# steventan0110/nFST

Measured on AMD Instinct MI355X. Metric: lattice-arcs/sec forward-backward (log-Z), higher is better.
Workload: dtype f32

## Files before the change

nfst_amd/csrc/fb_kernels.h:

```cpp
#pragma once

struct LdsPlan {
  int rows2, v2, v4;
  __host__ __device__ LdsPlan(int max_rows, int vocab)
      : rows2((max_rows + 1) & ~1), v2((vocab + 3) & ~1), v4((vocab + 3) & ~3) {}
  __host__ __device__ int64_t fb_fixed_precise() const {
    return ((int64_t)2 * rows2 + v2) * 16 + (int64_t)v4 * 4 + 2 * kSweepFlags * 4 + 2048;
  }
  __host__ __device__ int64_t bwd_fixed_precise() const { return ((int64_t)rows2 + v2) * 16 + kSweepFlags * 4 + 1024; }
  static __host__ __device__ int64_t sweep_words(int R, int RS) { return (int64_t)R * kSlotWords + (int64_t)RS * kRawWords; }
  __host__ __device__ int64_t fb_bytes(int R, int RS) const {
    return ((int64_t)2 * rows2 + v2) * 8 + (int64_t)v4 * 4 + 2 * sweep_words(R, RS) * 4 + 2 * kSweepFlags * 4 + 1024;
  }
  __host__ __device__ int64_t bwd_bytes(int R, int RS) const {
    return ((int64_t)rows2 + v2) * 8 + sweep_words(R, RS) * 4 + kSweepFlags * 4;
  }
};


template <int NT, int EXTRA, bool TW = false, bool PREC = false>
__global__ __launch_bounds__(NT) void k_backward(nfst_batch lat, nfst_scores sc, int R, int RS, float *logbeta,
                                                 double *logz64, float *logz32, float2 *beta_me) {
  static_assert(!PREC || TW, "precise flavour: tile waves");
  typedef typename ValOf<PREC>::T VT;
  extern __shared__ float2 lds_raw[];
  VT *lds = reinterpret_cast<VT *>(lds_raw);
  const int b = blockIdx.x, tid = threadIdx.x, lane = tid & 63;
  if (lat.only && lat.only[b] != lat.only_tag) return;
  const float theta_first = tid < lat.vocab ? sc.theta[(size_t)sc.theta_stride * b + tid] : 0.0f;
  const Meta m = load_meta(lat.meta, b);
  const LdsPlan plan(lat.max_rows, lat.vocab);
  VT *beta = lds;
  VT *th = lds + plan.rows2;
  uint32_t *ring = (uint32_t *)(th + plan.v2);
  const Extra ex{lat.weighted ? lat.arc_w : nullptr, sc.arc_scores};
  const int wv = __builtin_amdgcn_readfirstlane(tid >> 6);
  uint32_t *raw = ring + (size_t)R * kSlotWords;
  constexpr int kTwSlot = PREC ? kSlotWordsP : kSlotWords2;
  const int32_t *bwd_perm = lat.bwd_perm + m.bwd_slot_off;
  constexpr bool kSelf = NT != 512;
  constexpr int kAhead = kSelf ? kDmaAheadShared : kDmaAheadDeep;
  constexpr int kNE = kSelf ? 2 : 4, kFirstX = kSelf ? 2 : 4;
  static_assert(!TW || NT == 512, "tile waves: the one-lattice-per-CU flavour");
  if (TW) {
  } else if (kSelf) {
    if (wv == 1) self_start<kAhead>(m.bwd_u, lat.bwd_stream + m.bwd_off, m.bwd_tiles, raw, lane);
  } else if (wv == 2) {
    loader_start(m.bwd_u, lat.bwd_stream + m.bwd_off, m.bwd_tiles, raw, RS, lane);
  }
  const bool x_wave = TW ? (wv == 1 || wv == 2 || wv == 3 || wv == 5) : (EXTRA != 0 && wv >= kFirstX);
  const int x_index = TW ? (wv < 4 ? wv - 1 : 3) : wv - kFirstX;
  WeightWave<8, kNE, EXTRA, TW, PREC> xw8;
  if (x_wave && m.bwd_u == 8) xw8.start_maps(lat.bwd_stream + m.bwd_off, bwd_perm, m.bwd_tiles, ex, x_index, lane);
  for (int i = tid; i < m.n_rows; i += NT) val_set(beta[i], 0.0f, kEZero);
  load_theta(th, sc.theta, sc.theta_stride, b, lat.vocab, tid, NT, theta_first);
  if (x_wave && m.bwd_u == 8) xw8.start_gathers(lane);
  __syncthreads();
  int *flags = (int *)(ring + (TW ? (int64_t)R * kTwSlot : LdsPlan::sweep_words(R, RS)));
  if (tid == 0) {
    val_set(beta[m.sink], 0.5f, 1);
    for (int i = 0; i < kSweepFlags; ++i) flags[i] = 0;
  }
  __syncthreads();
  const bool tw_v2 = TW && m.bwd_wide == 0;
  if (x_wave) {
    run_weights<kNE, EXTRA, TW, PREC>(xw8, m.bwd_u, lat.bwd_stream + m.bwd_off, bwd_perm, m.bwd_tiles, ex, x_index, ring, R, flags,
                                      (const float2 *)th, (const float2 *)beta, tw_v2, lds_addr(flags + kSweepFlags) + lane * (PREC ? 16 : 8), 0u, 0, lane);
  } else if constexpr (TW) {
    if (wv == 0) {
      __builtin_amdgcn_s_setprio(3);
      if constexpr (PREC) tile_sweep2p<kNE>(m.bwd_tiles, ring, R, flags, flags + 4, lane);
      else if (tw_v2) tile_sweep2<4, kNE>(m.bwd_tiles, ring, R, flags, flags + 4, lane);
      else tile_sweep<4, true, kNE>(m.bwd_tiles, ring, R, flags, flags + 4, lane);
      __builtin_amdgcn_s_setprio(0);
    }
  } else if (wv < (kSelf ? 2 : 3))
    run_sweep<EXTRA, kSelf, kAhead, kNE>(wv, m.bwd_u, m.bwd_wide != 0, raw, RS, lat.bwd_stream + m.bwd_off,
              m.bwd_tiles, ring, R, flags, (float2 *)beta, (const float2 *)th, lane);
  __syncthreads();
  if (tid == 0) {
    const double z = me_log64(beta[0]);
    if (logz64) logz64[b] = z;
    if (logz32) logz32[b] = (float)z;
  }
  for (int i = tid; i < m.n_rows; i += NT) {
    if (logbeta) logbeta[m.row_off + i] = me_log32(beta[i]);
    if (beta_me) beta_me[m.row_off + i] = me_f2(beta[i]);
  }
}

__device__ __forceinline__ void exp_me_fast(float extra, float &m, int &e) {
  const float x = fminf(fmaxf(extra, -1.0e8f), 9.0e7f);
  const float kf = rintf(x * 1.44269504088896341f);
  float t = fmaf(-kf, 0.693145751953125f, x);
  t = fmaf(-kf, 1.42860682030941723e-6f, t);
  m = __builtin_amdgcn_exp2f(t * 1.44269504088896341f);
  e = (int)kf;
}
__device__ __forceinline__ float arc_posterior(const float2 av, const float2 bv, const float2 tw, float rz,
                                               int ez, bool has_extra, float mx, int ex) {
  float mw = tw.x;
  int ew = __float_as_int(tw.y);
  if (has_extra) {
    mw *= mx;
    ew += ex;
  }
  const float mm = (av.x * mw) * (bv.x * rz);
  const int ee = __float_as_int(av.y) + ew + __float_as_int(bv.y) - ez;
  return ldexpf(mm, max(ee, -300));
}

template <int NT, int EXTRA, bool FUSED = false, bool TW = false, bool PREC = false>
__global__ __launch_bounds__(NT) void k_forward_backward(
    nfst_batch lat, nfst_scores sc, int R, int RS, float *__restrict__ logalpha, float *__restrict__ logbeta,
    double *__restrict__ logz64, float *__restrict__ logz32, double *__restrict__ logz_total, int total_slot,
    float *__restrict__ posterior,
    float *__restrict__ grad_theta, float2 *__restrict__ beta_me) {
  static_assert(!PREC || (TW && EXTRA != 3), "precise flavour: tile waves, per-arc extras from HBM / L2");
  typedef typename ValOf<PREC>::T VT;
  extern __shared__ float2 lds_raw[];
  VT *lds = reinterpret_cast<VT *>(lds_raw);
  constexpr int kTwSlot = PREC ? kSlotWordsP : kSlotWords2;
  const int b = blockIdx.x, tid = threadIdx.x, lane = tid & 63;
  if (lat.only && lat.only[b] != lat.only_tag) return;
  if (tid == 0) NFST_STAMP(0);
  const float theta_first = tid < lat.vocab ? sc.theta[(size_t)sc.theta_stride * b + tid] : 0.0f;
  const Meta m = load_meta(lat.meta, b);
  const LdsPlan plan(lat.max_rows, lat.vocab);
  VT *alpha = lds;
  VT *beta = lds + plan.rows2;
  VT *th = lds + 2 * plan.rows2;
  float *gth = (float *)(th + plan.v2);
  uint32_t *ring = (uint32_t *)(gth + plan.v4);
  const Extra ex{lat.weighted ? lat.arc_w : nullptr, sc.arc_scores};
  constexpr bool has_extra = EXTRA != 0;
  constexpr bool kCached = EXTRA == 3;
  static_assert(!kCached || TW, "staged extras: tile-wave kernels");
  static_assert(!TW || (NT == 1024 && !FUSED), "tile waves: the one-lattice-per-CU flavour");
  const int wv = __builtin_amdgcn_readfirstlane(tid >> 6);
  const bool bwd_side = (wv & 1) == 0;
  const uint32_t *my_prog = bwd_side ? lat.bwd_stream + m.bwd_off : lat.fwd_stream + m.fwd_off;
  const int32_t *my_perm = bwd_side ? lat.bwd_perm + m.bwd_slot_off : lat.fwd_perm + m.fwd_slot_off;
  const int my_tiles = bwd_side ? m.bwd_tiles : m.fwd_tiles;
  const int my_u = bwd_side ? m.bwd_u : m.fwd_u;
  const bool my_wide = (bwd_side ? m.bwd_wide : m.fwd_wide) != 0;
  uint32_t *my_ring = bwd_side ? ring : ring + (TW ? (int64_t)R * kTwSlot : LdsPlan::sweep_words(R, RS));
  const bool tw_v2 = TW && !my_wide;
  uint32_t *my_raw = my_ring + (size_t)R * kSlotWords;
  constexpr bool kSelf = NT != 1024;
  constexpr int kAhead = kSelf ? kDmaAheadShared : kDmaAheadDeep;
  static_assert(!(FUSED && EXTRA), "the fused sweep takes no per-arc extras");
  static_assert(!(EXTRA && NT < 512), "the extras waves need idle waves: 512 threads at least");
  constexpr int kNE = (TW || NT == 1024) ? 4 : 2, kFirstX = NT == 1024 ? 8 : 4;
  const bool x_wave = TW ? (wv >= 2 && wv < 10) : EXTRA != 0 && wv >= kFirstX;
  const int x_index = TW ? (wv - 2) >> 1 : (wv - kFirstX) >> 1;
  if (FUSED) {
    if (wv < 2) FusedSweep<false>::start(my_prog, my_tiles, lane);
  } else if (TW) {
  } else if (kSelf) {
    if (wv == 2 || wv == 3) self_start<kAhead>(my_u, my_prog, my_tiles, my_raw, lane);
  } else if (wv == 6 || wv == 7) {
    loader_start(my_u, my_prog, my_tiles, my_raw, RS, lane);
  }
  WeightWave<8, kNE, EXTRA, TW, PREC> xw8;
  if (x_wave && my_u == 8) xw8.start_maps(my_prog, my_perm, my_tiles, ex, x_index, lane);
  for (int i = tid; i < m.n_rows; i += NT) {
    val_set(alpha[i], 0.0f, kEZero);
    val_set(beta[i], 0.0f, kEZero);
  }
  load_theta(th, sc.theta, sc.theta_stride, b, lat.vocab, tid, NT, theta_first);
  if (grad_theta) for (int l = tid; l < lat.vocab; l += NT) gth[l] = 0.0f;
  if (x_wave && my_u == 8) xw8.start_gathers(lane);
  __syncthreads();
  int *flags = (int *)(ring + 2 * (TW ? (int64_t)R * kTwSlot : LdsPlan::sweep_words(R, RS)));
  float *xc = (float *)(flags + 2 * kSweepFlags + 256);
  constexpr int kTrash = PREC ? 16 : 8;
  const int xc_first = m.arc_off & ~3;
  if (kCached) {
    const int a_lo = m.arc_off, a_hi = m.arc_off + m.n_arcs;
    for (int a = xc_first + 4 * tid; a < a_hi; a += 4 * NT) {
      float4 x = make_float4(0.0f, 0.0f, 0.0f, 0.0f);
      if (a >= a_lo && a + 4 <= a_hi) {
        if (ex.arc_w) x = *reinterpret_cast<const float4 *>(ex.arc_w + a);
        if (ex.arc_scores) {
          const float4 y = *reinterpret_cast<const float4 *>(ex.arc_scores + a);
          x.x += y.x; x.y += y.y; x.z += y.z; x.w += y.w;
        }
      } else {
        float t[4] = {0.0f, 0.0f, 0.0f, 0.0f};
        for (int q = 0; q < 4; ++q)
          if (a + q >= a_lo && a + q < a_hi) t[q] = ex.at(a + q);
        x = make_float4(t[0], t[1], t[2], t[3]);
      }
      *reinterpret_cast<float4 *>(xc + (a - xc_first)) = x;
    }
  }
  if (tid == 0) {
    val_set(beta[m.sink], 0.5f, 1);
    val_set(alpha[0], 0.5f, 1);
    for (int i = 0; i < 2 * kSweepFlags; ++i) flags[i] = 0;
  }
  __syncthreads();
  if (tid == 0) NFST_STAMP(1);
  const bool want_post = posterior != nullptr || grad_theta != nullptr;
  const int a_begin = m.arc_off, a_end = m.arc_off + m.n_arcs;
  const int v_begin = (a_begin + 3) & ~3, v_end = a_end & ~3;
  constexpr int kSweepThreads = 256;
  constexpr int kHelpers = NT - kSweepThreads;
  constexpr int kPre = (kHelpers > 0) ? 7 : 0;
  uint4 psd[kPre > 0 ? kPre : 1];
  uint2 plb[kPre > 0 ? kPre : 1];
  float4 pxm[kPre > 0 ? kPre : 1];
  int4 pxe[kPre > 0 ? kPre : 1];
  auto extras4 = [&](int a) {
    float4 x = make_float4(0.0f, 0.0f, 0.0f, 0.0f);
    if (kCached) return *reinterpret_cast<const float4 *>(xc + (a - xc_first));
    if (has_extra) {
      if (ex.arc_w) x = *reinterpret_cast<const float4 *>(ex.arc_w + a);
      if (ex.arc_scores) {
        const float4 y = *reinterpret_cast<const float4 *>(ex.arc_scores + a);
        x.x += y.x; x.y += y.y; x.z += y.z; x.w += y.w;
      }
    }
    return x;
  };
  auto preload_arcs = [&]() {
#pragma unroll
    for (int u = 0; u < kPre; ++u) {
      const int a = v_begin + 4 * (u * kHelpers + (tid - kSweepThreads));
      if (a < v_end) {
        psd[u] = *reinterpret_cast<const uint4 *>(lat.arc_sd + a);
        plb[u] = *reinterpret_cast<const uint2 *>(lat.arc_l16 + a);
        if (has_extra) pxm[u] = extras4(a);
      }
    }
    if (has_extra) {
#pragma unroll
      for (int u = 0; u < kPre; ++u) {
        const float4 x = pxm[u];
        exp_me_fast(x.x, pxm[u].x, pxe[u].x); exp_me_fast(x.y, pxm[u].y, pxe[u].y);
        exp_me_fast(x.z, pxm[u].z, pxe[u].z); exp_me_fast(x.w, pxm[u].w, pxe[u].w);
      }
    }
  };
  if constexpr (FUSED) {
    if (wv < 2) {
      const uint32_t trash = lds_addr(flags + 2 * kSweepFlags) + (bwd_side ? 0 : 512) + lane * 8;
      if (my_wide) FusedSweep<true>::run(my_prog, my_tiles, (const float2 *)(bwd_side ? beta : alpha), (const float2 *)th, trash, lane);
      else FusedSweep<false>::run(my_prog, my_tiles, (const float2 *)(bwd_side ? beta : alpha), (const float2 *)th, trash, lane);
    }
  } else if (x_wave) {
    run_weights<kNE, EXTRA, TW, PREC>(xw8, my_u, my_prog, my_perm, my_tiles, ex, x_index, my_ring, R, bwd_side ? flags : flags + kSweepFlags,
                                      (const float2 *)th, (const float2 *)(bwd_side ? beta : alpha), tw_v2,
                                      lds_addr(flags + 2 * kSweepFlags) + (bwd_side ? 0 : 64 * kTrash) + lane * kTrash, lds_addr(xc), xc_first, lane);
    if (TW && wv == 2) NFST_STAMP(6);
  } else if constexpr (TW) {
    if (wv < 2) {
      int *fl = bwd_side ? flags : flags + kSweepFlags;
      __builtin_amdgcn_s_setprio(3);
      if constexpr (PREC) tile_sweep2p<kNE>(my_tiles, my_ring, R, fl, fl + 4, lane);
      else if (tw_v2) tile_sweep2<4, kNE>(my_tiles, my_ring, R, fl, fl + 4, lane, bwd_side ? 5 : -1);
      else tile_sweep<4, true, kNE>(my_tiles, my_ring, R, fl, fl + 4, lane);
      __builtin_amdgcn_s_setprio(0);
      NFST_STAMP(bwd_side ? 2 : 3);
    }
  } else if (wv < 4 || (!kSelf && (wv == 6 || wv == 7))) {
    run_sweep<EXTRA, kSelf, kAhead, kNE>(wv < 4 ? wv >> 1 : 2, my_u, my_wide, my_raw, RS, my_prog,
                     my_tiles, my_ring, R, bwd_side ? flags : flags + kSweepFlags, (float2 *)(bwd_side ? beta : alpha), (const float2 *)th, lane);
  }
  if (kPre > 0 && want_post && tid >= kSweepThreads) preload_arcs();
  __syncthreads();
  if (tid == 0) NFST_STAMP(4);
  const float2 zme = me_f2(beta[0]);
  if (tid == 0) {
    const double z = me_log64(beta[0]);
    if (logz64) logz64[b] = z;
    if (logz_total) {
      atomicAdd(&logz_total[total_slot], z);
      if (b == 0) logz_total[(total_slot + 1) % 3] = 0.0;
    }
    if (logz32) logz32[b] = (float)z;
  }
  const float rz = (zme.x > 0.0f) ? 1.0f / zme.x : 0.0f;
  const int ez = __float_as_int(zme.y);
  auto do_group = [&](const uint4 sd, const uint2 lb, int a, const float4 xm, const int4 xe) {
    const float xmv[4] = {xm.x, xm.y, xm.z, xm.w};
    const int xev[4] = {xe.x, xe.y, xe.z, xe.w};
    const uint32_t sdv[4] = {sd.x, sd.y, sd.z, sd.w};
    const int ll[4] = {(int)(lb.x & 0xffffu), (int)(lb.x >> 16), (int)(lb.y & 0xffffu), (int)(lb.y >> 16)};
    float pp[4];
#pragma unroll
    for (int q = 0; q < 4; ++q) {
      const int s0 = (int)(sdv[q] & 0xffffu), d0 = (int)(sdv[q] >> 16);
      pp[q] = (s0 != d0) ? arc_posterior(me_f2(alpha[s0]), me_f2(beta[d0]), me_f2(th[ll[q]]), rz, ez, has_extra, xmv[q], xev[q]) : 0.0f;
      if (grad_theta && pp[q] > 0.0f) atomicAdd(&gth[ll[q]], pp[q]);
    }
    if (posterior) {
      typedef float f4v __attribute__((ext_vector_type(4)));
      __builtin_nontemporal_store(f4v{pp[0], pp[1], pp[2], pp[3]}, reinterpret_cast<f4v *>(posterior + a));
    }
  };
  if (kPre > 0 && tid >= kSweepThreads && want_post) {
#pragma unroll
    for (int u = 0; u < kPre; ++u) {
      const int a = v_begin + 4 * (u * kHelpers + (tid - kSweepThreads));
      if (a < v_end) do_group(psd[u], plb[u], a, pxm[u], pxe[u]);
    }
  }
  for (int i = tid; i < m.n_rows; i += NT) {
    if (logalpha) __builtin_nontemporal_store(me_log32(alpha[i]), logalpha + m.row_off + i);
    if (logbeta) __builtin_nontemporal_store(me_log32(beta[i]), logbeta + m.row_off + i);
    if (beta_me) beta_me[m.row_off + i] = me_f2(beta[i]);
  }
  if (want_post) {
    constexpr int kPB = 4;
    for (int a0 = v_begin + 4 * (kPre * kHelpers + tid); a0 < v_end; a0 += NT * 4 * kPB) {
      uint4 sd[kPB];
      uint2 lb[kPB];
      float4 xe[kPB];
#pragma unroll
      for (int u = 0; u < kPB; ++u) {
        const int a = min(a0 + u * NT * 4, v_end - 4);
        sd[u] = *reinterpret_cast<const uint4 *>(lat.arc_sd + a);
        lb[u] = *reinterpret_cast<const uint2 *>(lat.arc_l16 + a);
        xe[u] = extras4(a);
      }
#pragma unroll
      for (int u = 0; u < kPB; ++u) {
        const int a = a0 + u * NT * 4;
        if (a >= v_end) break;
        float4 gm = make_float4(1.0f, 1.0f, 1.0f, 1.0f);
        int4 ge = make_int4(0, 0, 0, 0);
        if (has_extra) {
          exp_me_fast(xe[u].x, gm.x, ge.x); exp_me_fast(xe[u].y, gm.y, ge.y);
          exp_me_fast(xe[u].z, gm.z, ge.z); exp_me_fast(xe[u].w, gm.w, ge.w);
        }
        do_group(sd[u], lb[u], a, gm, ge);
      }
    }
    const int n_head = min(v_begin, a_end) - a_begin;
    const int n_tail = (v_end >= v_begin) ? a_end - v_end : 0;
    if (tid < n_head + n_tail) {
      const int a = tid < n_head ? a_begin + tid : v_end + (tid - n_head);
      const int s0 = lat.arc_src[a], d0 = lat.arc_dst[a], l0 = lat.arc_label[a];
      float hm = 1.0f;
      int he = 0;
      if (has_extra) exp_me_fast(kCached ? xc[a - xc_first] : ex.at(a), hm, he);
      const float p = (s0 != d0) ? arc_posterior(me_f2(alpha[s0]), me_f2(beta[d0]), me_f2(th[l0]), rz, ez, has_extra, hm, he) : 0.0f;
      if (posterior) posterior[a] = p;
      if (grad_theta && p > 0.0f) atomicAdd(&gth[l0], p);
    }
    if (grad_theta) {
      __syncthreads();
      float *gout = grad_theta + (size_t)b * lat.vocab;
      for (int l = tid; l < lat.vocab; l += NT) gout[l] = gth[l];
    }
  }
#ifdef NFST_PROF
  __syncthreads();
  if (tid == 0) NFST_STAMP(7);
#endif
}
```

nfst_amd/csrc/tile_pipeline.h:

```cpp
#pragma once

constexpr int kDmaAheadDeep = 8, kRawSlotsDeep = 12, kDmaAheadShared = 4, kRawSlotsShared = kDmaAheadShared + 1;
constexpr int kRawWords = 64 * (1 + 4);
constexpr int kSlotWords = 64 * (1 + 3 * 4);
constexpr int kSlotWords2 = 1024;
constexpr int kSlotWordsP = 1280;
constexpr int kPreciseTiles = 192;
constexpr int kMaxRing = 12, kMinRing = 3;

template <int CTRL>
__device__ __forceinline__ int dpp_i(int v) {
  return __builtin_amdgcn_update_dpp(0, v, CTRL, 0xf, 0xf, false);
}
template <int CTRL>
__device__ __forceinline__ float dpp_f(float v) {
  return __int_as_float(__builtin_amdgcn_update_dpp(0, __float_as_int(v), CTRL, 0xf, 0xf, false));
}

template <int STAGES>
__device__ __forceinline__ int seg_max(int Em, int g) {
  if (STAGES >= 1) { const int o = dpp_i<0xB1>(Em); Em = (g >= 1) ? max(Em, o) : Em; }
  if (STAGES >= 2) { const int o = dpp_i<0x4E>(Em); Em = (g >= 2) ? max(Em, o) : Em; }
  if (STAGES >= 3) { const int o = dpp_i<0x141>(Em); Em = (g >= 3) ? max(Em, o) : Em; }
  if (STAGES >= 4) { const int o = dpp_i<0x140>(Em); Em = (g >= 4) ? max(Em, o) : Em; }
// ... 837 lines not shown
}

constexpr int kSweepFlags = 8;
template <int EXTRA, bool SELF, int AHEAD, int NE>
__device__ __forceinline__ void run_sweep(int role, int U, bool wide, uint32_t *raw, int RS, const uint32_t *g,
                                          int n_tiles, uint32_t *ring, int R, int *flags,
                                          float2 *val, const float2 *th, int lane) {
  int *prog = flags, *land = flags + 1, *rland = flags + 2, *xland = flags + 4;
  if (role == 0) {
    if (U == 8) U = 4;
    if (wide) {
      if (U == 4) tile_sweep<4, true>(n_tiles, ring, R, prog, land, lane);
      else if (U == 2) tile_sweep<2, true>(n_tiles, ring, R, prog, land, lane);
      else tile_sweep<1, true>(n_tiles, ring, R, prog, land, lane);
    } else {
      if (U == 4) tile_sweep<4, false>(n_tiles, ring, R, prog, land, lane);
      else if (U == 2) tile_sweep<2, false>(n_tiles, ring, R, prog, land, lane);
      else tile_sweep<1, false>(n_tiles, ring, R, prog, land, lane);
    }
  } else if (role == 1) {
    if (U == 8) tile_decoder<8, EXTRA, SELF, AHEAD>(n_tiles, raw, RS, rland, g, xland, NE, ring, R, prog, land, val, th, lane);
    else if (U == 4) tile_decoder<4, EXTRA, SELF, AHEAD>(n_tiles, raw, RS, rland, g, xland, NE, ring, R, prog, land, val, th, lane);
    else if (U == 2) tile_decoder<2, EXTRA, SELF, AHEAD>(n_tiles, raw, RS, rland, g, xland, NE, ring, R, prog, land, val, th, lane);
    else tile_decoder<1, EXTRA, SELF, AHEAD>(n_tiles, raw, RS, rland, g, xland, NE, ring, R, prog, land, val, th, lane);
  } else if (role == 2) {
    if (!SELF) {
      if (U == 8) tile_loader<8, AHEAD>(g, n_tiles, raw, RS, land, rland, lane);
      else if (U == 4) tile_loader<4, AHEAD>(g, n_tiles, raw, RS, land, rland, lane);
      else if (U == 2) tile_loader<2, AHEAD>(g, n_tiles, raw, RS, land, rland, lane);
      else tile_loader<1, AHEAD>(g, n_tiles, raw, RS, land, rland, lane);
    }
  }
}

template <int U>
struct Dec2 {
  uint32_t dst;
  float k0, k1, k2;
  uint32_t opa[U];
  v2f tw[U];
};
template <int U>
__device__ __forceinline__ void dec2_fetch(uint32_t sb, int lane, Dec2<U> &d) {
  const v4u h = *(const lds_v4u *)(uintptr_t)(sb + lane * 16);
  d.dst = h.x; d.k0 = __uint_as_float(h.y); d.k1 = __uint_as_float(h.z); d.k2 = __uint_as_float(h.w);
  if (U == 4) {
    const v4u a = *(const lds_v4u *)(uintptr_t)(sb + 1024 + lane * 16);
    const v4f p = *(const lds_v4f *)(uintptr_t)(sb + 2048 + lane * 16);
    const v4f q = *(const lds_v4f *)(uintptr_t)(sb + 3072 + lane * 16);
    d.opa[0] = a.x; d.opa[1 % U] = a.y; d.opa[2 % U] = a.z; d.opa[3 % U] = a.w;
    d.tw[0] = v2f{p.x, p.y}; d.tw[1 % U] = v2f{p.z, p.w}; d.tw[2 % U] = v2f{q.x, q.y}; d.tw[3 % U] = v2f{q.z, q.w};
  } else if (U == 2) {
    const v2u a = *(const lds_v2u *)(uintptr_t)(sb + 1024 + lane * 8);
    const v4f p = *(const lds_v4f *)(uintptr_t)(sb + 2048 + lane * 16);
    d.opa[0] = a.x; d.opa[1 % U] = a.y;
    d.tw[0] = v2f{p.x, p.y}; d.tw[1 % U] = v2f{p.z, p.w};
  } else {
    d.opa[0] = *(const lds_u32 *)(uintptr_t)(sb + 1024 + lane * 4);
    d.tw[0] = *(const lds_v2f *)(uintptr_t)(sb + 2048 + lane * 8);
  }
}
template <int U>
__device__ __forceinline__ void tile_math2(const v2f (&tw)[U], const v2f (&vv)[U], const Dec2<U> &c, int &ref) {
  const int nref = -ref;
  float mt[U];
  int d[U];
#pragma unroll
  for (int j = 0; j < U; ++j) {
    mt[j] = tw[j].x * vv[j].x;
    d[j] = __float_as_int(tw[j].y) + __float_as_int(vv[j].y) + nref;
  }
  int dmax = d[0];
#pragma unroll
  for (int j = 1; j < U; ++j) dmax = max(dmax, d[j]);
  float M = ldexpf(mt[0], d[0]);
#pragma unroll
  for (int j = 1; j < U; ++j) M += ldexpf(mt[j], d[j]);
  constexpr int kZeroish = -(1 << 27);
  const bool bad = ((uint32_t)(dmax + 64) > 128u) & (dmax > kZeroish);
  int E = ref;
  const int e0 = __builtin_amdgcn_readfirstlane(dmax);
  const int ref_old = ref;
  ref = (e0 > kZeroish) ? e0 + ref_old : ref_old;
  if (__builtin_expect(__builtin_amdgcn_ballot_w64(bad) != 0, 0)) {
    M = ldexpf(mt[0], d[0] - dmax);
#pragma unroll
    for (int j = 1; j < U; ++j) M += ldexpf(mt[j], d[j] - dmax);
    E = dmax + ref_old;
    const uint64_t m0 = __builtin_amdgcn_ballot_w64(c.k0 != 0.0f), m1 = __builtin_amdgcn_ballot_w64(c.k1 != 0.0f),
                   m2 = __builtin_amdgcn_ballot_w64(c.k2 != 0.0f);
    seg_reduce_exec<3>(M, E, m0, m1, m2);
  } else {
    asm volatile(
        "s_nop 1\n\t"
        "v_fmac_f32_dpp %[m], %[m], %[k0] quad_perm:[1,0,3,2] row_mask:0xf bank_mask:0xf\n\t"
        "s_nop 1\n\t"
        "v_fmac_f32_dpp %[m], %[m], %[k1] quad_perm:[2,3,0,1] row_mask:0xf bank_mask:0xf\n\t"
        "s_nop 1\n\t"
        "v_fmac_f32_dpp %[m], %[m], %[k2] row_half_mirror row_mask:0xf bank_mask:0xf"
        : [m] "+v"(M)
        : [k0] "v"(c.k0), [k1] "v"(c.k1), [k2] "v"(c.k2));
    E = (M == 0.0f) ? kEZero : E;
  }
  const float2 r = me_pack(M, E);
  *(lds_v2f *)(uintptr_t)c.dst = v2f{r.x, r.y};
}

template <int U>
__device__ __forceinline__ int tile_math3(const Dec2<U> &c, const v2f (&vv)[U], const int ref) {
  const int nref = -ref;
  float mt[U];
  int d[U];
#pragma unroll
  for (int j = 0; j < U; ++j) {
    mt[j] = c.tw[j].x * vv[j].x;
    asm("v_add3_u32 %0, %1, %2, %3" : "=v"(d[j]) : "v"(__float_as_int(c.tw[j].y)), "v"(__float_as_int(vv[j].y)), "s"(nref));
  }
  int dmax = d[0];
#pragma unroll
  for (int j = 1; j < U; ++j) dmax = max(dmax, d[j]);
  constexpr int kZeroish = -(1 << 27);
  const uint64_t bad = __builtin_amdgcn_ballot_w64(((uint32_t)(dmax + 64) > 128u) & (dmax > kZeroish));
  const int ref_old = ref;
  float M = ldexpf(mt[0], d[0]);
#pragma unroll
  for (int j = 1; j < U; ++j) M += ldexpf(mt[j], d[j]);
  asm volatile(
      "s_nop 1\n\t"
      "v_fmac_f32_dpp %[m], %[m], %[k0] quad_perm:[1,0,3,2] row_mask:0xf bank_mask:0xf\n\t"
      "s_nop 1\n\t"
      "v_fmac_f32_dpp %[m], %[m], %[k1] quad_perm:[2,3,0,1] row_mask:0xf bank_mask:0xf\n\t"
      "s_nop 1\n\t"
      "v_fmac_f32_dpp %[m], %[m], %[k2] row_half_mirror row_mask:0xf bank_mask:0xf"
      : [m] "+v"(M)
      : [k0] "v"(c.k0), [k1] "v"(c.k1), [k2] "v"(c.k2));
  int E = ref_old;
  if (__builtin_expect(bad != 0, 0)) {
    M = ldexpf(mt[0], d[0] - dmax);
#pragma unroll
    for (int j = 1; j < U; ++j) M += ldexpf(mt[j], d[j] - dmax);
    E = dmax + ref_old;
    const uint64_t m0 = __builtin_amdgcn_ballot_w64(c.k0 != 0.0f), m1 = __builtin_amdgcn_ballot_w64(c.k1 != 0.0f),
                   m2 = __builtin_amdgcn_ballot_w64(c.k2 != 0.0f);
    seg_reduce_exec<3>(M, E, m0, m1, m2);
  }
  int ex;
  const float mant = frexpf(M, &ex);
  const int eo = (M != 0.0f) ? max(E + ex, kEZero) : kEZero;
  *(lds_v2f *)(uintptr_t)c.dst = v2f{mant, __int_as_float(eo)};
  return dmax;
}

#ifdef NFST_PROF
__device__ unsigned long long fb_prof[4096 * 8];
#define NFST_STAMP(k) do { if ((threadIdx.x & 63) == 0 && blockIdx.x < 4096) fb_prof[blockIdx.x * 8 + (k)] = wall_clock64(); } while (0)
#else
#define NFST_STAMP(k) do { } while (0)
#endif
template <int U, int NEF>
__device__ __forceinline__ void tile_sweep2(int n_tiles, const uint32_t *ring, int R, int *prog, const int *land, int lane, int prof_slot = -1) {
  static_assert(NEF == 4, "four tile waves per sweep");
  (void)prof_slot;
  if (n_tiles <= 0) return;
  constexpr uint32_t SB = kSlotWords2 * 4;
  const uint32_t ring_base = lds_addr(ring), ring_end = ring_base + (uint32_t)R * SB;
  const uint32_t land_a = lds_addr(land), prog_a = lds_addr(prog);
  auto flags_now = [&]() { return *(const volatile lds_v4u *)(uintptr_t)land_a; };
  auto margin_x = [](const v4u f) { return min(min((int)f.y - 1, (int)f.z - 2), (int)f.w - 3); };
  auto margin_y = [](const v4u f) { return (int)f.x - 4; };
  auto wait_group = [&](int T, int which) {
    for (;;) {
      const v4u f = flags_now();
      if (__builtin_amdgcn_readfirstlane(which ? margin_y(f) : margin_x(f)) > T) break;
      __builtin_amdgcn_s_sleep(1);
    }
    asm volatile("" ::: "memory");
  };
  while (__builtin_amdgcn_readfirstlane((int)*(const volatile lds_u32 *)(uintptr_t)land_a) <= 0) __builtin_amdgcn_s_sleep(1);
  asm volatile("" ::: "memory");
#ifdef NFST_PROF
  if (prof_slot >= 0) NFST_STAMP(prof_slot);
#endif
  uint32_t gbase = ring_base;
  v4u margin = {0u, 0u, 0u, 0u}, margin1 = {0u, 0u, 0u, 0u};
  int ref = 0;
  int dmax0 = 0;
  Dec2<U> da, db;
  dec2_fetch<U>(gbase, lane, da);
  asm volatile("" ::: "memory");
#define NFST_S2_STEP(K, CUR, NXT)                                                                          \
  {                                                                                                       \
    v2f vv[U];                                                                                            \
    _Pragma("unroll") for (int j = 0; j < U; ++j) vv[j] = *(const lds_v2f *)(uintptr_t)CUR.opa[j];         \
    asm volatile("" ::: "memory");                                                                        \
    __builtin_amdgcn_sched_barrier(0);          \
    if (K == 3) {                                                                                         \
      gbase = (gbase + 4 * SB == ring_end) ? ring_base : gbase + 4 * SB;                                  \
      asm volatile("" ::"v"(margin1));                                                                    \
      if (__builtin_expect(__builtin_amdgcn_readfirstlane(margin_y(margin1)) <= T, 0)) wait_group(T, 1);     \
    }                                                                                                     \
    dec2_fetch<U>(gbase + (K == 3 ? 0u : (K + 1) * SB), lane, NXT);                                       \
    if (K == 1) margin1 = flags_now();                                                                     \
    if (K == 3) margin = flags_now();                                                        \
    asm volatile("" ::: "memory");                                                                        \
    __builtin_amdgcn_sched_barrier(0);                                                                    \
    const int dm_ = tile_math3<U>(CUR, vv, ref);                                                          \
    if (K == 0) dmax0 = dm_;                                                                              \
    if (K & 1) *(volatile lds_u32 *)(uintptr_t)prog_a = (uint32_t)(T + K + 2);  \
    asm volatile("" ::: "memory");                                                                        \
    __builtin_amdgcn_sched_barrier(0);                                                                    \
  }
  int T = 0;
  for (; T + 4 <= n_tiles; T += 4) {
    asm volatile("" ::"v"(margin));
    if (__builtin_expect(__builtin_amdgcn_readfirstlane(margin_x(margin)) <= T, 0)) wait_group(T, 0);
    NFST_S2_STEP(0, da, db)
    NFST_S2_STEP(1, db, da)
    NFST_S2_STEP(2, da, db)
    NFST_S2_STEP(3, db, da)
    const int e0 = __builtin_amdgcn_readfirstlane(dmax0);
    ref = __builtin_amdgcn_readfirstlane((e0 > -(1 << 27)) ? e0 + ref : ref);
  }
  if (T < n_tiles) {
    asm volatile("" ::"v"(margin));
    if (__builtin_expect(__builtin_amdgcn_readfirstlane(margin_x(margin)) <= T, 0)) wait_group(T, 0);
    NFST_S2_STEP(0, da, db)
    if (T + 1 < n_tiles) {
      NFST_S2_STEP(1, db, da)
      if (T + 2 < n_tiles) NFST_S2_STEP(2, da, db)
    }
  }
#undef NFST_S2_STEP
}

struct Dec2P {
  uint32_t dst;
  uint32_t k0, k1, k2;
  uint32_t opa[4];
  double wm[4];
  int we[4];
};
__device__ __forceinline__ void dec2p_fetch(uint32_t sb, int lane, Dec2P &d) {
  const v4u h = *(const lds_v4u *)(uintptr_t)(sb + lane * 16);
  const v4u a = *(const lds_v4u *)(uintptr_t)(sb + 1024 + lane * 16);
  const v4u p = *(const lds_v4u *)(uintptr_t)(sb + 2048 + lane * 16);
  const v4u q = *(const lds_v4u *)(uintptr_t)(sb + 3072 + lane * 16);
  const v4u e = *(const lds_v4u *)(uintptr_t)(sb + 4096 + lane * 16);
  d.dst = h.x; d.k0 = h.y; d.k1 = h.z; d.k2 = h.w;
  d.opa[0] = a.x; d.opa[1] = a.y; d.opa[2] = a.z; d.opa[3] = a.w;
  d.wm[0] = __hiloint2double((int)p.y, (int)p.x); d.wm[1] = __hiloint2double((int)p.w, (int)p.z);
  d.wm[2] = __hiloint2double((int)q.y, (int)q.x); d.wm[3] = __hiloint2double((int)q.w, (int)q.z);
  d.we[0] = (int)e.x; d.we[1] = (int)e.y; d.we[2] = (int)e.z; d.we[3] = (int)e.w;
}
template <int CTRL>
__device__ __forceinline__ double dpp_d(double v) {
  return __hiloint2double(__builtin_amdgcn_update_dpp(0, __double2hiint(v), CTRL, 0xf, 0xf, false),
                          __builtin_amdgcn_update_dpp(0, __double2loint(v), CTRL, 0xf, 0xf, false));
}
template <int STAGES>
__device__ __forceinline__ double seg_sum64(double M, int g) {
  if (STAGES >= 1) { const double o = dpp_d<0xB1>(M); M = (g >= 1) ? M + o : M; }
  if (STAGES >= 2) { const double o = dpp_d<0x4E>(M); M = (g >= 2) ? M + o : M; }
  if (STAGES >= 3) { const double o = dpp_d<0x141>(M); M = (g >= 3) ? M + o : M; }
  if (STAGES >= 4) { const double o = dpp_d<0x140>(M); M = (g >= 4) ? M + o : M; }
  if (STAGES >= 5) { const double o = __shfl_xor(M, 16); M = (g >= 5) ? M + o : M; }
  if (STAGES >= 6) { const double o = __shfl_xor(M, 32); M = (g >= 6) ? M + o : M; }
  return M;
}
__device__ __forceinline__ double ldexp_clamped(double m, int d) {
  return ldexp(m, max(d, -2000));
}
__device__ __forceinline__ int tile_math3p(const Dec2P &c, const Rec64 (&vv)[4], const int ref) {
  const int nref = -ref;
  double mt[4];
  int d[4];
#pragma unroll
  for (int j = 0; j < 4; ++j) {
    mt[j] = c.wm[j] * vv[j].m;
    asm("v_add3_u32 %0, %1, %2, %3" : "=v"(d[j]) : "v"(c.we[j]), "v"(vv[j].e), "s"(nref));
  }
  int dmax = d[0];
#pragma unroll
  for (int j = 1; j < 4; ++j) dmax = max(dmax, d[j]);
  constexpr int kZeroish = -(1 << 27);
  const uint32_t wide = (c.dst >> 25) & 1u;
  const uint64_t bad = __builtin_amdgcn_ballot_w64((((uint32_t)(dmax + 900) > 1800u) & (dmax > kZeroish)) | (wide != 0));
  double M = ldexp(mt[0], d[0]);
#pragma unroll
  for (int j = 1; j < 4; ++j) M += ldexp(mt[j], d[j]);
  {
    int plo, phi;
#define NFST_DPP_PAIR(CTRL)                                                                                              \
    asm volatile("s_nop 1\n\tv_mov_b32_dpp %0, %2 " CTRL " row_mask:0xf bank_mask:0xf\n\tv_mov_b32_dpp %1, %3 " CTRL      \
                 " row_mask:0xf bank_mask:0xf" : "=&v"(plo), "=&v"(phi) : "v"(__double2loint(M)), "v"(__double2hiint(M)))
    NFST_DPP_PAIR("quad_perm:[1,0,3,2]");
    M = fma(__hiloint2double(phi, plo), __hiloint2double((int)c.k0, 0), M);
    NFST_DPP_PAIR("quad_perm:[2,3,0,1]");
    M = fma(__hiloint2double(phi, plo), __hiloint2double((int)c.k1, 0), M);
    NFST_DPP_PAIR("row_half_mirror");
    M = fma(__hiloint2double(phi, plo), __hiloint2double((int)c.k2, 0), M);
#undef NFST_DPP_PAIR
  }
  int E = ref;
  if (__builtin_expect(bad != 0, 0)) {
    const int g = (int)ctl_g(c.dst);
    M = ldexp_clamped(mt[0], d[0] - dmax);
#pragma unroll
    for (int j = 1; j < 4; ++j) M += ldexp_clamped(mt[j], d[j] - dmax);
// ... 145 lines not shown
```

profiles/tune/chunk_stamps.py:

```python
import ctypes as C, os, sys
sys.path.insert(0, os.path.dirname(os.path.dirname(os.path.dirname(os.path.abspath(__file__)))))
import numpy as np, torch
from nfst_amd import ops, synth, _lib
from nfst_amd.lattice import LatticeBatch
B = int(sys.argv[1]) if len(sys.argv) > 1 else 64
dev = torch.device("cuda")
if len(sys.argv) > 2 and sys.argv[2] == "narrow":
    sys.path.insert(0, os.path.dirname(os.path.abspath(__file__)))
    rng = np.random.default_rng(8000)
    lats = [synth.layered_lattice(8000 + i, n_states=int(rng.integers(400, 1501)), avg_degree=float(rng.choice([3.0, 5.0])), vocab=250,
                                  width=int(rng.choice([1, 2, 3])), span=int(rng.choice([1, 2])), max_degree=40) for i in range(B)]
else:
    lats = synth.snips_shaped_batch(B, vocab=250)
host = LatticeBatch.from_synth(lats)
assert host.build_chunks(force=True)
lat = host.to(dev)
theta = torch.from_numpy(synth.label_scores(1, 250, mean=-1.5, std=0.8)).to(dev)
for _ in range(5):
    r = ops.forward_backward(lat, theta)
torch.cuda.synchronize()
raw = C.CDLL(_lib.LIB_PATH)
n = 2 * B
buf = np.zeros(n * 8, np.uint64)
assert raw.nfst_prof_read(buf.ctypes.data_as(C.c_void_p), n * 8) == 0
t = buf.reshape(n, 8).astype(np.int64)
own = (t[:, 1:5] - t[:, :4]) / 100.0
rel_end = (t[:, 4] - t[:, 0].min()) / 100.0
m = lat.chunks.meta_host.reshape(n, 8)
tab = lat.chunks._t["tab"].cpu().numpy().reshape(-1, 4)
longest = np.array([tab[m[i, 4]:m[i, 4] + m[i, 0], 2].max() for i in range(n)])
print("us per phase (median / max over workgroups): weights+init %.1f / %.1f, pass 1 %.1f / %.1f, pass 2 %.1f / %.1f, pass 3 %.1f / %.1f; last end %.1f" %
      (np.median(own[:, 0]), own[:, 0].max(), np.median(own[:, 1]), own[:, 1].max(), np.median(own[:, 2]), own[:, 2].max(),
       np.median(own[:, 3]), own[:, 3].max(), rel_end.max()))
print("pass 1: ns per entry of the longest chunk: median %.0f min %.0f max %.0f" % tuple(np.percentile(own[:, 1] * 1e3 / longest, [50, 0, 100])))
print("pass 2: ns per chunk: median %.0f; by F:" % np.median(own[:, 2] * 1e3 / m[:, 0]),
      {int(F): round(float(np.median((own[:, 2] * 1e3 / m[:, 0])[m[:, 1] == F]))) for F in np.unique(m[:, 1])})
slow = np.argsort(rel_end)[-4:]
print("slowest:", [(int(i), "C %d F %d R %d longest %d" % (m[i, 0], m[i, 1], m[i, 2], longest[i]), [round(float(x), 1) for x in own[i]]) for i in slow])
```

profiles/tune/stamps.py:

```python
import ctypes as C, os, sys
sys.path.insert(0, os.path.dirname(os.path.dirname(os.path.dirname(os.path.abspath(__file__)))))
import numpy as np, torch
from nfst_amd import ops, synth, _lib
from nfst_amd.lattice import LatticeBatch
B = int(sys.argv[1]) if len(sys.argv) > 1 else 256
rot = int(sys.argv[2]) if len(sys.argv) > 2 else 4
dev = torch.device("cuda")
lats = [LatticeBatch.from_synth(synth.bench_batch(B, first_seed=1234 + 100000 * r), device=dev) for r in range(rot)]
theta = torch.from_numpy(synth.label_scores(1, 256)).to(dev)
outs = [None] * rot
for it in range(10 * rot + 1):
    r = it % rot
    outs[r] = ops.forward_backward(lats[r], theta, out=outs[r])
torch.cuda.synchronize()
raw = C.CDLL(_lib.LIB_PATH)
buf = np.zeros(B * 8, np.uint64)
assert raw.nfst_prof_read(buf.ctypes.data_as(C.c_void_p), B * 8) == 0
t = buf.reshape(B, 8).astype(np.int64)
rel = (t - t[:, 0].min()) / 100.0
lat = lats[0]
tiles = np.maximum(lat.meta_host[:, _lib.META_BWD_TILES], lat.meta_host[:, _lib.META_FWD_TILES])
names = ["entry", "init done", "beta swept", "alpha swept", "barrier", "first tile", "tile wave 0 done", "end"]
print(f"B={B}, {rot} batches rotating: us since the first workgroup entered (min / median / max over workgroups)")
for i in (0, 1, 5, 6, 2, 3, 4, 7):
    print(f"  {names[i]:18s} {rel[:, i].min():8.2f} {np.median(rel[:, i]):8.2f} {rel[:, i].max():8.2f}")
own = (t - t[:, :1]) / 100.0
print("  per workgroup, since its own entry: init %.2f, first tile %.2f, sweeps done %.2f, barrier -> end %.2f (medians)" %
      (np.median(own[:, 1]), np.median(own[:, 5]), np.median(np.maximum(own[:, 2], own[:, 3])), np.median(own[:, 7] - own[:, 4])))
dur = (np.maximum(t[:, 2], t[:, 3]) - t[:, 5]) / 100.0
print("  sweep duration / tile (ns): min %.0f median %.0f max %.0f;  tiles: min %d median %d max %d" %
      (*np.percentile(dur / tiles * 1e3, [0, 50, 100]), tiles.min(), np.median(tiles), tiles.max()))
slow = np.argsort(rel[:, 7])[-4:]
print("  slowest workgroups (id, tiles, first tile, swept, end):", [(int(b), int(tiles[b]), round(float(rel[b, 5]), 2), round(float(max(rel[b, 2], rel[b, 3])), 2), round(float(rel[b, 7]), 2)) for b in slow])
```

Measured before the change: 131.0 billion.

## Use buffer stores for outputs, vectorize row logs, rebalance sweep/helper threads

Posterior and log-alpha/log-beta outputs now go through raw buffer-resource 128-bit stores with a streaming cache policy. The row log outputs are written four at a time with an aligned head and tail, and the alpha and beta rows start at different thread offsets. The fused kernel also reserves 128 instead of 256 threads for the sweep, giving more threads to posterior preloading with 6 prefetched groups each. Extra profiling stamps are added. Risks: fewer sweep-side threads may slow the sweep phase, and buffer bounds or alignment handling could be wrong at row edges.

```diff
diff --git a/nfst_amd/csrc/fb_kernels.h b/nfst_amd/csrc/fb_kernels.h
--- a/nfst_amd/csrc/fb_kernels.h
+++ b/nfst_amd/csrc/fb_kernels.h
@@ -86,6 +86,36 @@
   for (int i = tid; i < m.n_rows; i += NT) {
     if (logbeta) logbeta[m.row_off + i] = me_log32(beta[i]);
     if (beta_me) beta_me[m.row_off + i] = me_f2(beta[i]);
+  }
+}
+
+typedef float f4v __attribute__((ext_vector_type(4)));
+struct OutBuf {
+  __amdgpu_buffer_rsrc_t rsrc;
+  __device__ __forceinline__ OutBuf(float *p, int n_floats) {
+    const uint64_t a = (uint64_t)(uintptr_t)p;
+    const uint32_t lo = __builtin_amdgcn_readfirstlane((uint32_t)a), hi = __builtin_amdgcn_readfirstlane((uint32_t)(a >> 32));
+    rsrc = __builtin_amdgcn_make_buffer_rsrc(reinterpret_cast<void *>((uintptr_t)(((uint64_t)hi << 32) | lo)), 0,
+                                             __builtin_amdgcn_readfirstlane(n_floats) * 4, 0x00020000);
+  }
+  __device__ __forceinline__ void store4(int i, const f4v v) const {
+    typedef uint32_t u4v __attribute__((ext_vector_type(4)));
+    __builtin_amdgcn_raw_buffer_store_b128(__builtin_bit_cast(u4v, v), rsrc, i * 4, 0, 16);
+  }
+};
+template <int NT, class VT>
+__device__ __forceinline__ void rows_out(float *out, const VT *val, int n, int tid, int first) {
+  const int head = min((int)((0u - (uint32_t)(uintptr_t)out) >> 2 & 3u), n);
+  const int groups = (n - head) >> 2, tail = head + 4 * groups;
+  const OutBuf ob(out, n);
+  for (int g = (tid - first) & (NT - 1); g < groups; g += NT) {
+    const int i = head + 4 * g;
+    ob.store4(i, f4v{me_log32(val[i]), me_log32(val[i + 1]), me_log32(val[i + 2]), me_log32(val[i + 3])});
+  }
+  const int t = (tid - first) & (NT - 1);
+  if (t < head + (n - tail)) {
+    const int i = t < head ? t : tail + (t - head);
+    __builtin_nontemporal_store(me_log32(val[i]), out + i);
   }
 }
 
@@ -205,9 +235,9 @@
   const bool want_post = posterior != nullptr || grad_theta != nullptr;
   const int a_begin = m.arc_off, a_end = m.arc_off + m.n_arcs;
   const int v_begin = (a_begin + 3) & ~3, v_end = a_end & ~3;
-  constexpr int kSweepThreads = 256;
+  constexpr int kSweepThreads = 128;
   constexpr int kHelpers = NT - kSweepThreads;
-  constexpr int kPre = (kHelpers > 0) ? 7 : 0;
+  constexpr int kPre = (NT > 256) ? 6 : 0;
   uint4 psd[kPre > 0 ? kPre : 1];
   uint2 plb[kPre > 0 ? kPre : 1];
   float4 pxm[kPre > 0 ? kPre : 1];
@@ -283,6 +313,7 @@
   }
   const float rz = (zme.x > 0.0f) ? 1.0f / zme.x : 0.0f;
   const int ez = __float_as_int(zme.y);
+  const OutBuf post_out(posterior ? posterior + a_begin : nullptr, posterior ? m.n_arcs : 0);
   auto do_group = [&](const uint4 sd, const uint2 lb, int a, const float4 xm, const int4 xe) {
     const float xmv[4] = {xm.x, xm.y, xm.z, xm.w};
     const int xev[4] = {xe.x, xe.y, xe.z, xe.w};
@@ -295,10 +326,7 @@
       pp[q] = (s0 != d0) ? arc_posterior(me_f2(alpha[s0]), me_f2(beta[d0]), me_f2(th[ll[q]]), rz, ez, has_extra, xmv[q], xev[q]) : 0.0f;
       if (grad_theta && pp[q] > 0.0f) atomicAdd(&gth[ll[q]], pp[q]);
     }
-    if (posterior) {
-      typedef float f4v __attribute__((ext_vector_type(4)));
-      __builtin_nontemporal_store(f4v{pp[0], pp[1], pp[2], pp[3]}, reinterpret_cast<f4v *>(posterior + a));
-    }
+    if (posterior) post_out.store4(a - a_begin, f4v{pp[0], pp[1], pp[2], pp[3]});
   };
   if (kPre > 0 && tid >= kSweepThreads && want_post) {
 #pragma unroll
@@ -307,11 +335,17 @@
       if (a < v_end) do_group(psd[u], plb[u], a, pxm[u], pxe[u]);
     }
   }
-  for (int i = tid; i < m.n_rows; i += NT) {
-    if (logalpha) __builtin_nontemporal_store(me_log32(alpha[i]), logalpha + m.row_off + i);
-    if (logbeta) __builtin_nontemporal_store(me_log32(beta[i]), logbeta + m.row_off + i);
-    if (beta_me) beta_me[m.row_off + i] = me_f2(beta[i]);
-  }
+#ifdef NFST_PROF
+  if (wv == 4) {
+    NFST_STAMP(8);
+    asm volatile("s_waitcnt vmcnt(0)" ::: "memory");
+    NFST_STAMP(9);
+  }
+#endif
+  if (logalpha) rows_out<NT>(logalpha + m.row_off, alpha, m.n_rows, tid, 0);
+  if (logbeta) rows_out<NT>(logbeta + m.row_off, beta, m.n_rows, tid, NT / 2);
+  if (beta_me) for (int i = tid; i < m.n_rows; i += NT) beta_me[m.row_off + i] = me_f2(beta[i]);
+  if (wv == 0) NFST_STAMP(10);
   if (want_post) {
     constexpr int kPB = 4;
     for (int a0 = v_begin + 4 * (kPre * kHelpers + tid); a0 < v_end; a0 += NT * 4 * kPB) {
diff --git a/nfst_amd/csrc/tile_pipeline.h b/nfst_amd/csrc/tile_pipeline.h
--- a/nfst_amd/csrc/tile_pipeline.h
+++ b/nfst_amd/csrc/tile_pipeline.h
@@ -1013,8 +1013,9 @@
 }
 
 #ifdef NFST_PROF
-__device__ unsigned long long fb_prof[4096 * 8];
-#define NFST_STAMP(k) do { if ((threadIdx.x & 63) == 0 && blockIdx.x < 4096) fb_prof[blockIdx.x * 8 + (k)] = wall_clock64(); } while (0)
+constexpr int kProfSlots = 16;
+__device__ unsigned long long fb_prof[4096 * kProfSlots];
+#define NFST_STAMP(k) do { if ((threadIdx.x & 63) == 0 && blockIdx.x < 4096) fb_prof[blockIdx.x * kProfSlots + (k)] = wall_clock64(); } while (0)
 #else
 #define NFST_STAMP(k) do { } while (0)
 #endif
diff --git a/profiles/tune/chunk_stamps.py b/profiles/tune/chunk_stamps.py
--- a/profiles/tune/chunk_stamps.py
+++ b/profiles/tune/chunk_stamps.py
@@ -21,9 +21,9 @@
 torch.cuda.synchronize()
 raw = C.CDLL(_lib.LIB_PATH)
 n = 2 * B
-buf = np.zeros(n * 8, np.uint64)
-assert raw.nfst_prof_read(buf.ctypes.data_as(C.c_void_p), n * 8) == 0
-t = buf.reshape(n, 8).astype(np.int64)
+buf = np.zeros(n * 16, np.uint64)
+assert raw.nfst_prof_read(buf.ctypes.data_as(C.c_void_p), n * 16) == 0
+t = buf.reshape(n, 16)[:, :8].astype(np.int64)
 own = (t[:, 1:5] - t[:, :4]) / 100.0
 rel_end = (t[:, 4] - t[:, 0].min()) / 100.0
 m = lat.chunks.meta_host.reshape(n, 8)
diff --git a/profiles/tune/stamps.py b/profiles/tune/stamps.py
--- a/profiles/tune/stamps.py
+++ b/profiles/tune/stamps.py
@@ -14,15 +14,17 @@
     outs[r] = ops.forward_backward(lats[r], theta, out=outs[r])
 torch.cuda.synchronize()
 raw = C.CDLL(_lib.LIB_PATH)
-buf = np.zeros(B * 8, np.uint64)
-assert raw.nfst_prof_read(buf.ctypes.data_as(C.c_void_p), B * 8) == 0
-t = buf.reshape(B, 8).astype(np.int64)
+SLOTS = 16
+buf = np.zeros(B * SLOTS, np.uint64)
+assert raw.nfst_prof_read(buf.ctypes.data_as(C.c_void_p), B * SLOTS) == 0
+t = buf.reshape(B, SLOTS).astype(np.int64)
 rel = (t - t[:, 0].min()) / 100.0
 lat = lats[0]
 tiles = np.maximum(lat.meta_host[:, _lib.META_BWD_TILES], lat.meta_host[:, _lib.META_FWD_TILES])
-names = ["entry", "init done", "beta swept", "alpha swept", "barrier", "first tile", "tile wave 0 done", "end"]
+names = ["entry", "init done", "beta swept", "alpha swept", "barrier", "first tile", "tile wave 0 done", "end",
+         "w4 stores issued", "w4 stores drained", "w0 rows issued"]
 print(f"B={B}, {rot} batches rotating: us since the first workgroup entered (min / median / max over workgroups)")
-for i in (0, 1, 5, 6, 2, 3, 4, 7):
+for i in (0, 1, 5, 6, 2, 3, 4, 10, 8, 9, 7):
     print(f"  {names[i]:18s} {rel[:, i].min():8.2f} {np.median(rel[:, i]):8.2f} {rel[:, i].max():8.2f}")
 own = (t - t[:, :1]) / 100.0
 print("  per workgroup, since its own entry: init %.2f, first tile %.2f, sweeps done %.2f, barrier -> end %.2f (medians)" %
@@ -32,3 +34,11 @@
       (*np.percentile(dur / tiles * 1e3, [0, 50, 100]), tiles.min(), np.median(tiles), tiles.max()))
 slow = np.argsort(rel[:, 7])[-4:]
 print("  slowest workgroups (id, tiles, first tile, swept, end):", [(int(b), int(tiles[b]), round(float(rel[b, 5]), 2), round(float(max(rel[b, 2], rel[b, 3])), 2), round(float(rel[b, 7]), 2)) for b in slow])
+tail = (t[:, [10, 8, 9, 7]] - t[:, 4:5]) / 100.0
+print("  tail since the workgroup's barrier (min / median / max):")
+for j, n in enumerate(("wave 0 rows issued", "wave 4 stores issued", "wave 4 stores drained", "end")):
+    print(f"    {n:22s} {tail[:, j].min():6.2f} {np.median(tail[:, j]):6.2f} {tail[:, j].max():6.2f}")
+print("    drain (stamp 9 - 8)    %6.2f %6.2f %6.2f;  end - drained %6.2f %6.2f %6.2f" %
+      (*np.percentile(tail[:, 2] - tail[:, 1], [0, 50, 100]), *np.percentile(tail[:, 3] - tail[:, 2], [0, 50, 100])))
+print("  slowest workgroups' tails (id, arcs, barrier, rows issued, stores issued, drained, end):",
+      [(int(b), int(lat.meta_host[b, _lib.META_N_ARCS]),*(round(float(rel[b, i]), 2) for i in (4, 10, 8, 9, 7))) for b in slow])
```

Result: slower. 126.5 billion (-3.5%).
